# for-the-juan/SpGEMM

Hardware: AMD Instinct MI355X
Metric: SpGEMM GFLOPS (fp64, C=A^2) + achieved HBM GB/s fraction, 1/2/4/8 MI355X (higher is better)
Workload: dtype f64

## Files before the change

### spgemm_amd/csrc/tsg_rows.hip

```cpp
#include "tsg_internal.h"
#include "tsg_dev_common.h"

#include <cstdio>
#include <cstdlib>

namespace tsg {

namespace {

constexpr int S16_MAX = 16;
constexpr int RS_MAX = 64;
constexpr int S16_U = 2, S64_U = 2;
constexpr int M0_CAP = 256, M0_RUNS = 62, M0_NT = 64;
constexpr int M1_CAP = 512, M1_RUNS = 124, M1_NT = 128;
constexpr int M2_CAP = 1024, M2_RUNS = 248, M2_NT = 256;
constexpr int M3_CAP = 2048, M3_RUNS = 504, M3_NT = 512;
constexpr int M4_CAP = 4096, M4_RUNS = 512, M4_NT = 1024;
constexpr int W_CH = 32768;
constexpr int NCLS = 8;
constexpr int DR_SMAX = 4096;
constexpr int DR_CH = 16384;
constexpr int DR_GR = 16;
constexpr int DR_GMAX = 8192;
constexpr int BIN_ROWS = 2048;
constexpr int RH_NT = 1024;
constexpr int RH_WORDS = 16384;
constexpr long long RH_SPAN = (long long)RH_WORDS * 64;
constexpr int RH_BLK = 512;
constexpr int RH_NBLK = RH_WORDS / RH_BLK;
constexpr int RH_NGRP = RH_WORDS / 4;
constexpr int RH_PPT = 16;
constexpr int OW_CH = RH_PPT * RH_NT;
constexpr int OW_CV = 2 * RH_WORDS;
constexpr int OW_RUNS = 2 * RH_NT;
static_assert(OW_CH <= RH_WORDS, "one-walk rows: a pass's values fit the bitmap's LDS");

__device__ __forceinline__ u32 lanes_below(u64 b) {
    return __builtin_amdgcn_mbcnt_hi((u32)(b >> 32), __builtin_amdgcn_mbcnt_lo((u32)b, 0u));
}
__device__ __forceinline__ int key_col(u64 k) { return (int)(k >> 32); }

}

#ifdef TSG_ROWS_PROF
__device__ unsigned long long g_rows_prof[3][256][12];
#define RP_INIT unsigned long long rp_acc[12] = {}, rp_t = wall_clock64();
#define RP(k)                                         \
    do {                                              \
        const unsigned long long _t = wall_clock64(); \
        rp_acc[k] += _t - rp_t;                       \
        rp_t = _t;                                    \
    } while (0)
#define RP_DONE(K)                                                          \
    do {                                                                    \
        if (threadIdx.x == 0)                                               \
            for (int _k = 0; _k < 12; ++_k) atomicAdd(&g_rows_prof[K][blockIdx.x & 255][_k], rp_acc[_k]); \
    } while (0)
#else
#define RP_INIT
#define RP(k) \
    do {      \
    } while (0)
#define RP_DONE(K) \
    do {           \
    } while (0)
#endif

struct RowsArgs {
    const int *rpA;
    const double *vA;
    const int2 *ebnd;
    const long long *E;
    const int *Bcol;
    const double *Bval;
    const int4 *list;
    int nrows;
    int *rnnz;
    int *Scol;
    double *Sval;
};

__device__ __forceinline__ void rows_counters_reset(RowsCounters *cls) {
    constexpr int N = sizeof(RowsCounters) / sizeof(int);
    if (blockIdx.x == 0 && threadIdx.x < N) reinterpret_cast<int *>(cls)[threadIdx.x] = 0;
}

__global__ __launch_bounds__(WG) void k_rows_entries(const int *ciA, long nnzA, const int *rpB, int2 *ebnd,
                                                     long long *E, RowsCounters *cls) {
    rows_counters_reset(cls);
    for (long a = (long)blockIdx.x * WG + threadIdx.x; a <= nnzA; a += (long)gridDim.x * WG) {
        if (a == nnzA) {
            E[a] = 0;
            break;
        }
        const int k = ciA[a], b0 = rpB[k], b1 = rpB[k + 1];
        ebnd[a] = make_int2(b0, b1);
        E[a] = b1 - b0;
    }
}

__global__ __launch_bounds__(WG) void k_rows_entries_sum(const int *ciA, long nnzA, const int *rpB, int2 *ebnd,
                                                         long long *E, RowsCounters *cls, long long *part) {
    __shared__ long long red[WAVES];
    const int tid = threadIdx.x;
    rows_counters_reset(cls);
    const long base = (long)blockIdx.x * SCAN_TILE;
    int kk[SCAN_ITEMS];
#pragma unroll
    for (int u = 0; u < SCAN_ITEMS; ++u) {
        const long a = base + u * WG + tid;
        kk[u] = a < nnzA ? ciA[a] : 0;
    }
    int b0[SCAN_ITEMS], b1[SCAN_ITEMS];
#pragma unroll
    for (int u = 0; u < SCAN_ITEMS; ++u) {
        const long a = base + u * WG + tid;
        b0[u] = a < nnzA ? rpB[kk[u]] : 0;
        b1[u] = a < nnzA ? rpB[kk[u] + 1] : 0;
    }
    long long sum = 0;
#pragma unroll
    for (int u = 0; u < SCAN_ITEMS; ++u) {
        const long a = base + u * WG + tid;
        if (a < nnzA) {
            ebnd[a] = make_int2(b0[u], b1[u]);
            E[a] = b1[u] - b0[u];
            sum += b1[u] - b0[u];
        } else if (a == nnzA) {
            E[a] = 0;
        }
    }
    sum = block_sum(sum, red);
    if (tid == 0) part[blockIdx.x] = sum;
}

__device__ __forceinline__ int row_class(long long P, int k) {
    if (P == 0) return -1;
    if (P <= S16_MAX && k <= S16_MAX) return 0;
    if (P <= RS_MAX && k <= RS_MAX) return 1;
    if (P <= M0_CAP && k <= M0_RUNS) return 2;
    if (P <= M1_CAP && k <= M1_RUNS) return 3;
    if (P <= M2_CAP && k <= M2_RUNS) return 4;
    if (P <= M3_CAP && k <= M3_RUNS) return 5;
    if (P <= M4_CAP && k <= M4_RUNS) return 6;
    return 7;
}

__global__ __launch_bounds__(WG) void k_rows_bin(const int *rpA, int m, const long long *E, const long long *Etot,
                                                 int *rnnz, int4 *lists, RowsCounters *cls, long long *soff,
                                                 const int *spart, int snb, int *sflag) {
    __shared__ int gb[NCLS];
    __shared__ long long red64[WAVES];
    constexpr int RPT = BIN_ROWS / WG;
    __shared__ int wcu[RPT][NCLS][WAVES];
    const int tid = threadIdx.x, lane = lane_id(), wv = wave_id();
    const int r0 = blockIdx.x * BIN_ROWS, r1 = min(m, r0 + BIN_ROWS);
    if (blockIdx.x == 0 && tid == 0) {
        cls->products = (unsigned long long)*Etot;
        rnnz[m] = 0;
    }
    if (blockIdx.x == 0 && spart) {
        long long v = 0;
#pragma unroll 8
        for (int i = tid; i < snb; i += WG) v += spart[i];
        v = block_sum(v, red64);
        if (tid == 0 && v != 0) __hip_atomic_store(sflag, 1, __ATOMIC_RELAXED, __HIP_MEMORY_SCOPE_SYSTEM);
    }
    long long hp = 0, pmax = 0, drp = 0, hubr = 0, hbig = 0;
    int cu[RPT];
    int ra0[RPT], ra1[RPT];
#pragma unroll
    for (int u = 0; u < RPT; ++u) {
        const int r = r0 + u * WG + tid;
        ra0[u] = r < r1 ? rpA[r] : 0;
        ra1[u] = r < r1 ? rpA[r + 1] : 0;
    }
    long long e0[RPT], e1[RPT];
#pragma unroll
    for (int u = 0; u < RPT; ++u) {
        e0[u] = E[ra0[u]];
        e1[u] = E[ra1[u]];
    }
#pragma unroll
    for (int u = 0; u < RPT; ++u) {
        const int r = r0 + u * WG + tid;
        cu[u] = -1;
        if (r >= r1) continue;
        const long long P = e1[u] - e0[u];
        const int c = row_class(P, ra1[u] - ra0[u]);
        soff[r] = e0[u];
        cu[u] = c;
        if (c < 0) rnnz[r] = 0;
        hp += c == NCLS - 1 ? P : 0;
        hbig += c == NCLS - 1 && P <= kRowsHubProducts && P > OW_CH ? P - OW_CH : 0;
        pmax = max(pmax, P);
        if (P > kRowsHubProducts) drp += P;
        if (c == NCLS - 1 && ra1[u] - ra0[u] > OW_RUNS) ++hubr;
    }
    hp = block_sum(hp, red64);
    drp = block_sum(drp, red64);
    hubr = block_sum(hubr, red64);
    hbig = block_sum(hbig, red64);
#pragma unroll
    for (int d = 32; d > 0; d >>= 1) pmax = max(pmax, __shfl_xor(pmax, d, 64));
    if (lane == 0) red64[wv] = pmax;
    __syncthreads();
    if (tid == 0) {
        for (int w = 1; w < WAVES; ++w) pmax = max(pmax, red64[w]);
        if (hp) atomicAdd(&cls->hprod, (unsigned long long)hp);
        if (pmax) atomicMax(&cls->pmax, (unsigned long long)pmax);
        if (drp) atomicAdd(&cls->hubprod, (unsigned long long)drp);
        if (hubr) atomicAdd(&cls->hk, (unsigned long long)hubr);
        if (hbig) atomicAdd(&cls->hbig, (unsigned long long)hbig);
    }
    u64 mine[RPT];
#pragma unroll
    for (int u = 0; u < RPT; ++u) {
        mine[u] = 0;
#pragma unroll
        for (int t = 0; t < NCLS; ++t) {
            const u64 bt = __ballot(cu[u] == t);
            if (cu[u] == t) mine[u] = bt;
            if (lane == 0) wcu[u][t][wv] = __popcll(bt);
        }
    }
    __syncthreads();
    if (tid < NCLS) {
        int run = 0;
        for (int u = 0; u < RPT; ++u)
            for (int w = 0; w < WAVES; ++w) {
                const int v = wcu[u][tid][w];
                wcu[u][tid][w] = run;
                run += v;
            }
        gb[tid] = run ? atomicAdd(&cls->ncls[tid], run) : 0;
    }
    __syncthreads();
#pragma unroll
    for (int u = 0; u < RPT; ++u) {
        const int c = cu[u];
        if (c >= 0) {
            const int r = r0 + u * WG + tid;
            lists[(long)c * m + gb[c] + wcu[u][c][wv] + lanes_below(mine[u])] = make_int4(r, ra0[u], ra1[u] - ra0[u], 0);
        }
    }
}

constexpr int OH_NT = 1024, OH_PER = 8, OH_MAX = OH_NT * OH_PER, OH_NB = 64;
__global__ __launch_bounds__(OH_NT) void k_rows_order_h(const long long *E, const int *nrows, int4 *list) {
    __shared__ int cnt[OH_NB];
    const int tid = threadIdx.x;
    const int n = *nrows;
    if (n < 2 || n > OH_MAX) return;
    if (tid < OH_NB) cnt[tid] = 0;
    __syncthreads();
    int4 r[OH_PER];
    int b[OH_PER];
#pragma unroll
    for (int u = 0; u < OH_PER; ++u) {
        const int i = u * OH_NT + tid;
        r[u] = i < n ? list[i] : make_int4(-1, 0, 0, 0);
    }
#pragma unroll
    for (int u = 0; u < OH_PER; ++u)
        if (r[u].x >= 0) {
            const long long P = E[r[u].y + r[u].z] - E[r[u].y];
            b[u] = OH_NB - 1 - (int)min((long long)OH_NB - 1, P >> 10);
            atomicAdd(&cnt[b[u]], 1);
        }
    __syncthreads();
    if (tid < 64) {
        const int v = cnt[tid];
        const int inc = wave_incl_scan_dpp(v);
        cnt[tid] = inc - v;
    }
    __syncthreads();
#pragma unroll
    for (int u = 0; u < OH_PER; ++u)
        if (r[u].x >= 0) list[atomicAdd(&cnt[b[u]], 1)] = r[u];
}

template <int J> __device__ __forceinline__ int row_bcast16(int v) {
    return __builtin_amdgcn_update_dpp(0, v, 0x150 | J, 0xf, 0xf, false);
}
template <int V> struct IntC { static constexpr int value = V; };
template <int J, int N, class F> __device__ __forceinline__ void static_for(F &&f) {
    if constexpr (J < N) {
        f(IntC<J>{});
        static_for<J + 1, N>(f);
    }
}

template <int G, int U>
__global__ __launch_bounds__(WG) void k_rows_small(RowsArgs g) {
    constexpr int RPW = 64 / G;
    __shared__ u64 sk[WAVES][U][64];
    __shared__ double sv[WAVES][U][64];
    const int lane = lane_id(), wv = wave_id(), sl = lane % G, gb = lane - sl;
    const int w0 = (blockIdx.x * WAVES + wv) * RPW * U;
    if (w0 >= g.nrows) return;
    int r[U], a0[U], k[U];
    bool live[U];
    long long base[U];
#pragma unroll
    for (int u = 0; u < U; ++u) {
        const int i = w0 + u * RPW + lane / G;
        live[u] = i < g.nrows;
        r[u] = 0, a0[u] = 0, k[u] = 0;
        if (live[u]) {
            const int4 e = g.list[i];
            r[u] = e.x;
            a0[u] = e.y;
            k[u] = e.z;
        }
    }
    int2 be[U];
    double av[U];
#pragma unroll
    for (int u = 0; u < U; ++u) {
        be[u] = make_int2(0, 0);
        av[u] = 0.0;
        base[u] = 0;
        if (live[u]) base[u] = g.E[a0[u]];
        if (sl < k[u]) {
            be[u] = g.ebnd[a0[u] + sl];
            av[u] = g.vA[a0[u] + sl];
        }
    }
    int P[U], pp[U];
    double ra[U];
#pragma unroll
    for (int u = 0; u < U; ++u) {
        const int len = be[u].y - be[u].x, bs = be[u].x;
        int inc = len;
        inc += dpp_mov<0x111, 0xf>(0, inc);
        inc += dpp_mov<0x112, 0xf>(0, inc);
        inc += dpp_mov<0x114, 0xf>(0, inc);
        inc += dpp_mov<0x118, 0xf>(0, inc);
        if constexpr (G == 64) {
            inc += dpp_mov<0x142, 0xa>(0, inc);
            inc += dpp_mov<0x143, 0xc>(0, inc);
        }
        const int roff = sl < k[u] ? inc - len : INT_MAX;
        int run = 0;
        if constexpr (G == 64) {
            P[u] = __shfl(inc, G - 1, G);
            for (int j = 1; j < k[u]; ++j) run = (__builtin_amdgcn_readlane(roff, j) <= sl) ? j : run;
        } else {
            static_assert(G == 16, "row broadcasts: 16-lane groups");
            P[u] = row_bcast16<15>(inc);
            static_for<1, 16>([&](auto jc) {
                constexpr int j = decltype(jc)::value;
                run = row_bcast16<j>(roff) <= sl ? j : run;
            });
        }
        const int rs = __shfl(roff, run, G), rb = __shfl(bs, run, G);
        ra[u] = __shfl(av[u], run, G);
        pp[u] = rb + sl - rs;
    }
    u64 key[U];
    double x[U];
#pragma unroll
    for (int u = 0; u < U; ++u) {
        key[u] = ~0ull;
        x[u] = 0.0;
        if (sl < P[u]) {
            key[u] = ((u64)(u32)g.Bcol[pp[u]] << 32) | (u32)sl;
            x[u] = g.Bval[pp[u]];
        }
    }
#pragma unroll
    for (int u = 0; u < U; ++u) {
        const u32 khi = (u32)(key[u] >> 32), klo = (u32)key[u];
        int rank = 0;
        if constexpr (G == 64) {
            for (int f = 0; f < P[u]; ++f) {
                const u64 kf = ((u64)(u32)__builtin_amdgcn_readlane((int)khi, f) << 32) |
                               (u32)__builtin_amdgcn_readlane((int)klo, f);
                rank += kf < key[u];
            }
        } else {
            const u64 ku = key[u];
            static_for<0, 16>([&](auto fc) {
                constexpr int f = decltype(fc)::value;
                const u64 kf = ((u64)(u32)row_bcast16<f>((int)khi) << 32) | (u32)row_bcast16<f>((int)klo);
                rank += kf < ku;
            });
        }
        if (sl < P[u]) {
            sk[wv][u][gb + rank] = key[u];
            sv[wv][u][gb + rank] = ra[u] * x[u];
        }
    }
    wave_lds_sync();
    const u64 gm = (G == 64 ? ~0ull : ((1ull << (G & 63)) - 1ull)) << gb;
#pragma unroll
    for (int u = 0; u < U; ++u) {
        int col = -1;
        bool head = false;
        if (sl < P[u]) {
            col = key_col(sk[wv][u][gb + sl]);
            head = sl == 0 || key_col(sk[wv][u][gb + sl - 1]) != col;
        }
        const u64 hb = __ballot(head) & gm;
        if (head) {
            double sm = sv[wv][u][gb + sl];
            for (int j = sl + 1; j < P[u] && key_col(sk[wv][u][gb + j]) == col; ++j) sm += sv[wv][u][gb + j];
            const long long o = base[u] + (long long)lanes_below(hb);
            g.Scol[o] = col;
            g.Sval[o] = sm;
        }
        if (live[u] && sl == 0) g.rnnz[r[u]] = __popcll(hb);
    }
}

template <int U, class T>
__device__ __forceinline__ void search_ilp(const T *a, int (&b)[U], int (&len)[U], const T (&key)[U],
                                           const bool (&ub)[U]) {
    for (;;) {
        bool more = false;
#pragma unroll
        for (int u = 0; u < U; ++u) more |= len[u] > 0;
        if (!more) break;
#pragma unroll
        for (int u = 0; u < U; ++u) {
            const int half = len[u] >> 1, idx = b[u] + half;
            const T v = a[len[u] > 0 ? idx : 0];
            const bool go = len[u] > 0 && (v < key[u] || (ub[u] && v == key[u]));
            b[u] = go ? idx + 1 : b[u];
            len[u] = go ? len[u] - half - 1 : half;
        }
    }
}

template <int D> __device__ __forceinline__ u32 lane_xor(u32 v) {
    if constexpr (D == 1) return (u32)__builtin_amdgcn_mov_dpp((int)v, 0xB1, 0xf, 0xf, false);
    else if constexpr (D == 2) return (u32)__builtin_amdgcn_mov_dpp((int)v, 0x4E, 0xf, 0xf, false);
    else if constexpr (D < 32) return (u32)__builtin_amdgcn_ds_swizzle((int)v, (D << 10) | 0x1f);
    else return (u32)__shfl_xor((int)v, D, 64);
}

__device__ __forceinline__ u32 minmax_sel(u32 a, u32 b, u32 sel) { return min(max(a, b), max(min(a, b), sel)); }
template <int B> __device__ __forceinline__ u32 bit_fill(u32 v) { return (u32)((int)(v << (31 - B)) >> 31); }
constexpr int ilog2_c(int v) { return v <= 1 ? 0 : 1 + ilog2_c(v >> 1); }

template <int K, int J> __device__ __forceinline__ void bitonic_stage(u32 (&x)[4], int lane) {
    if constexpr (J >= 4) {
        constexpr int D = J / 4;
        u32 w = (u32)lane;
        if constexpr (K < 256) w ^= bit_fill<ilog2_c(K / 4)>((u32)lane);
        const u32 sel = bit_fill<ilog2_c(D)>(w);
#pragma unroll
        for (int u = 0; u < 4; ++u) x[u] = minmax_sel(x[u], lane_xor<D>(x[u]), sel);
    } else {
#pragma unroll
        for (int u = 0; u < 4; ++u)
            if ((u & J) == 0) {
                if constexpr (K < 4 || K >= 256) {
                    const bool asc = K < 4 ? (u & K) == 0 : true;
                    const u32 lo = min(x[u], x[u + J]), hi = max(x[u], x[u + J]);
                    x[u] = asc ? lo : hi;
                    x[u + J] = asc ? hi : lo;
                } else {
                    const u32 desc = bit_fill<ilog2_c(K / 4)>((u32)lane);
                    const u32 a = x[u], b = x[u + J];
                    x[u] = minmax_sel(a, b, desc);
                    x[u + J] = minmax_sel(a, b, ~desc);
                }
            }
    }
}
template <int K, int J> __device__ __forceinline__ void bitonic_merge(u32 (&x)[4], int lane) {
    bitonic_stage<K, J>(x, lane);
    if constexpr (J > 1) bitonic_merge<K, J / 2>(x, lane);
}
template <int K> __device__ __forceinline__ void bitonic_sort(u32 (&x)[4], int lane) {
    if constexpr (K > 2) bitonic_sort<K / 2>(x, lane);
    bitonic_merge<K, K / 2>(x, lane);
}
__device__ __forceinline__ void wave_sort256(u32 (&x)[4], int lane, int live) {
    bitonic_sort<64>(x, lane);
    if (live > 64) bitonic_merge<128, 64>(x, lane);
    if (live > 128) bitonic_merge<256, 128>(x, lane);
}

template <int STRIDE>
__device__ __forceinline__ int xwave_merge(u32 (&x)[4], u32 *kb, int lane, int wv, int P, int npow) {
    constexpr int SEG = 256;
    wv = __builtin_amdgcn_readfirstlane(wv);
    npow = __builtin_amdgcn_readfirstlane(npow);
    const int nlive = (__builtin_amdgcn_readfirstlane(P) + SEG - 1) / SEG;
    const bool live = wv < nlive;
    const int e0 = wv * SEG + 4 * lane;
    int src = 0;
    auto cmpx = [&](int pw, int off, bool rev) {
        if (pw >= nlive) return;
        const uint4 y = *reinterpret_cast<const uint4 *>(kb + src * STRIDE + off);
        const u32 yy[4] = {rev ? y.w : y.x, rev ? y.z : y.y, rev ? y.y : y.z, rev ? y.x : y.w};
        const u32 sel = pw < wv ? ~0u : 0u;
#pragma unroll
        for (int u = 0; u < 4; ++u) x[u] = minmax_sel(x[u], yy[u], sel);
    };
    for (int K = 2 * SEG; K <= npow; K <<= 1) {
        if (live) cmpx(wv ^ (K / SEG - 1), e0 ^ (K - 4), true);
        for (int J = K >> 2; J >= SEG; J >>= 1) {
            src ^= 1;
            if (live) *reinterpret_cast<uint4 *>(kb + src * STRIDE + e0) = make_uint4(x[0], x[1], x[2], x[3]);
            __syncthreads();
            if (live) cmpx(wv ^ (J / SEG), e0 ^ J, false);
        }
        if (live) bitonic_merge<256, 128>(x, lane);
        src ^= 1;
        if (live) *reinterpret_cast<uint4 *>(kb + src * STRIDE + e0) = make_uint4(x[0], x[1], x[2], x[3]);
        __syncthreads();
    }
    return src;
}

template <int NT, int CAP, int RUNS>
__global__ __launch_bounds__(NT, NT == 1024 ? 8 : 1) void k_rows_merge(RowsArgs g) {
    constexpr int NW = NT / 64;
    constexpr int IPM = (CAP + NT - 1) / NT | 1;
    constexpr int IB = CAP == 256 ? 8 : CAP == 512 ? 9 : CAP == 1024 ? 10 : CAP == 2048 ? 11 : 12;
    static_assert((1 << IB) == CAP, "CAP: a power of two in [256, 4096]");
    constexpr int SEG = 256;
    static_assert(CAP == 4 * NT, "four positions per thread");
    static_assert(RUNS <= NT, "a thread per A entry");
    __shared__ __align__(16) u32 kp[2][2][CAP];
    __shared__ int roff[RUNS + 1];
    __shared__ int rbs[RUNS];
    __shared__ double rav[RUNS];
    __shared__ int red[2 * NW];
    RP_INIT
    const int tid = threadIdx.x, lane = lane_id(), wv = wave_id();
    const int4 le = g.list[blockIdx.x];
    int2 be = make_int2(0, 0);
    double av = 0.0;
    if (tid < le.z) {
        be = g.ebnd[le.y + tid];
        av = g.vA[le.y + tid];
    }
    const long long base = g.E[le.y];
    double *const V = reinterpret_cast<double *>(kp[1][0]);
    {
        const int r = le.x;
        int k = 0, P = 0;
        {
            const int len = be.y - be.x;
            const u64 b = __ballot(len > 0);
            const int inc = wave_incl_scan_dpp(len);
            if (lane == 63) {
                red[wv] = __popcll(b);
                red[NW + wv] = inc;
            }
            __syncthreads();
            int off = 0, loff = 0;
#pragma unroll
            for (int w = 0; w < NW; ++w) {
                off += w < wv ? red[w] : 0;
                k += red[w];
                loff += w < wv ? red[NW + w] : 0;
                P += red[NW + w];
            }
            if (len > 0) {
                const int d = off + lanes_below(b);
                roff[d] = loff + inc - len;
                rbs[d] = be.x;
                rav[d] = av;
            }
            if (tid == 0) roff[k] = P;
            __syncthreads();
        }
        RP(0);
        const int e0 = wv * SEG + 4 * lane, ne = max(0, min(4, P - e0));
        int c[4] = {0, 0, 0, 0};
        u32 py[4] = {0, 0, 0, 0};
        double xv[4] = {0.0, 0.0, 0.0, 0.0};
        {
            int j = 0;
            if (ne > 0) j = lower_bound_dev(roff, 0, k + 1, e0 + 1) - 1;
            int pa[4] = {0, 0, 0, 0};
            double ra[4] = {0.0, 0.0, 0.0, 0.0}, bv[4] = {0.0, 0.0, 0.0, 0.0};
#pragma unroll
            for (int u = 0; u < 4; ++u)
                if (u < ne) {
                    const int q = e0 + u;
                    while (roff[j + 1] <= q) ++j;
                    pa[u] = rbs[j] + q - roff[j];
                    py[u] = ((u32)j << 16) | (u32)(q - roff[j]);
                    ra[u] = rav[j];
                }
#pragma unroll
            for (int u = 0; u < 4; ++u)
                if (u < ne) {
                    c[u] = g.Bcol[pa[u]];
                    bv[u] = g.Bval[pa[u]];
                }
#pragma unroll
            for (int u = 0; u < 4; ++u) xv[u] = u < ne ? ra[u] * bv[u] : 0.0;
        }
        int clo = INT_MAX, chi = -1;
#pragma unroll
        for (int u = 0; u < 4; ++u)
            if (u < ne) {
                clo = min(clo, c[u]);
                chi = max(chi, c[u]);
            }
        clo = wave_last(wave_incl_dpp(clo, INT_MAX, OpMin{}));
        chi = wave_last(wave_incl_dpp(chi, INT_MIN, OpMax{}));
        if (lane == 0) {
            red[wv] = clo;
            red[NW + wv] = chi;
        }
        __syncthreads();
        clo = red[0];
        chi = red[NW];
#pragma unroll
        for (int w = 1; w < NW; ++w) {
            clo = min(clo, red[w]);
            chi = max(chi, red[NW + w]);
        }
        const bool packed = (u32)(chi - clo) < (1u << (32 - IB)) - 1u;
        int npow = SEG;
        while (npow < P) npow <<= 1;
        u32 x[4] = {~0u, ~0u, ~0u, ~0u};
        if (packed) {
#pragma unroll
            for (int u = 0; u < 4; ++u) x[u] = u < ne ? ((u32)(c[u] - clo) << IB) | (u32)(e0 + u) : ~0u;
            if (ne > 0) {
                reinterpret_cast<double4 *>(V)[e0 >> 2] = make_double4(xv[0], xv[1], xv[2], xv[3]);
            }
            const int live = __builtin_amdgcn_readfirstlane(P - wv * SEG);
            if (live > 0) {
                wave_sort256(x, lane, live);
                *reinterpret_cast<uint4 *>(kp[0][0] + e0) = make_uint4(x[0], x[1], x[2], x[3]);
            }
        } else {
#pragma unroll
            for (int u = 0; u < 4; ++u)
                if (u < ne) {
                    kp[0][0][e0 + u] = (u32)c[u];
                    kp[0][1][e0 + u] = py[u];
                }
        }
        __syncthreads();
        RP(1);
        int src = 0;
        if (packed) src = xwave_merge<CAP>(x, kp[0][0], lane, wv, P, npow);
        const int ipt = ((P + NT - 1) / NT) | 1;
        const int q0 = min(P, tid * ipt), q1 = min(P, q0 + ipt), nq = q1 - q0;
        if (!packed) {
            const int *const bd = roff;
            const int nb = k;
            int j0 = 0;
            if (nq > 0) j0 = lower_bound_dev(roff, 0, k + 1, q0 + 1) - 1;
            for (int lw = 0; (1 << lw) < nb; ++lw) {
                const u32 *ik = kp[src][0], *ip = kp[src][1];
                u32 *ok = kp[src ^ 1][0], *op = kp[src ^ 1][1];
                int pr = j0 >> (lw + 1);
                for (int q = q0; q < q1;) {
                    while (bd[min((pr + 1) << (lw + 1), nb)] <= q) ++pr;
                    const int ps = bd[pr << (lw + 1)];
                    const int pm = bd[min((2 * pr + 1) << lw, nb)];
                    const int pe = bd[min((pr + 1) << (lw + 1), nb)];
                    const int la = pm - ps, lb = pe - pm, qq = q - ps;
                    int lo = max(0, qq - lb), hi = min(qq, la);
                    while (lo < hi) {
                        const int t = (lo + hi) >> 1;
                        if (ik[ps + t] <= ik[pm + qq - t - 1]) lo = t + 1; else hi = t;
                    }
                    int ia = lo, ib = qq - lo;
                    u32 ka = ia < la ? ik[ps + ia] : ~0u, kbv = ib < lb ? ik[pm + ib] : ~0u;
                    const int qe = min(q1, pe);
                    for (; q < qe; ++q) {
                        const bool ta = ka <= kbv;
                        ok[q] = ta ? ka : kbv;
                        op[q] = ta ? ps + ia : pm + ib;
                        ia += ta;
                        ib += !ta;
                        const u32 kn = ik[ta ? ps + ia : pm + ib];
                        const bool live = ta ? ia < la : ib < lb;
                        ka = ta ? (live ? kn : ~0u) : ka;
                        kbv = ta ? kbv : (live ? kn : ~0u);
                    }
                }
#pragma unroll
                for (int u = 0; u < IPM; ++u)
                    if (u < nq) op[q0 + u] = ip[op[q0 + u]];
                __syncthreads();
                src ^= 1;
            }
        }
        RP(2);
        int nh = 0;
        const int np = packed ? max(0, min(4, P - e0)) : 0;
        double xs[4] = {0.0, 0.0, 0.0, 0.0};
        u32 hd = 0;
        const u32 *const sk = packed ? kp[0][src] : kp[src][0];
        double *const vb = reinterpret_cast<double *>(kp[src ^ 1][0]);
        if (packed) {
            const u32 prev = e0 > 0 && np > 0 ? sk[e0 - 1] : ~0u;
#pragma unroll
            for (int u = 0; u < 4; ++u)
                if (u < np) {
                    xs[u] = V[x[u] & (CAP - 1)];
                    const u32 pk = u ? x[u - 1] : prev;
                    hd |= (e0 + u == 0 || (x[u] >> IB) != (pk >> IB)) ? 1u << u : 0u;
                }
            nh = __popc(hd);
        } else {
            const u32 *sp = kp[src][1];
            int pa[IPM] = {};
            double ra[IPM] = {};
#pragma unroll
            for (int u = 0; u < IPM; ++u)
                if (u < nq) {
                    const u32 key = sk[q0 + u];
                    const u32 pj = sp[q0 + u];
                    const int ru = (int)(pj >> 16);
                    pa[u] = rbs[ru] + (int)(pj & 0xffffu);
                    ra[u] = rav[ru];
                    nh += (q0 + u == 0 || key != sk[q0 + u - 1]);
                }
            double xx[IPM] = {};
#pragma unroll
            for (int u = 0; u < IPM; ++u)
                if (u < nq) xx[u] = ra[u] * g.Bval[pa[u]];
#pragma unroll
            for (int u = 0; u < IPM; ++u)
                if (u < nq) vb[q0 + u] = xx[u];
        }
        const int inc = wave_incl_scan_dpp(nh);
        if (lane == 63) red[wv] = inc;
        __syncthreads();
        RP(3);
        int o = inc - nh, tot = 0;
#pragma unroll
        for (int w = 0; w < NW; ++w) {
            o += w < wv ? red[w] : 0;
            tot += red[w];
        }
        if (tid == 0) g.rnnz[r] = tot;
        if (packed) {
#pragma unroll
            for (int u = 0; u < 4; ++u)
                if (hd >> u & 1u) {
                    const u32 col = x[u] >> IB;
// ... 1730 lines not shown
```

Baseline: 120.0.

## Use in-register bitonic sort on packed 32-bit keys for small-row SpGEMM

In the small-row kernel, products are now sorted by column with a register bitonic network over 32-bit keys. Each key packs the column offset from the group minimum with the lane index, and the network replaces the O(P) rank-counting loop over 64-bit keys. If the group's column span does not fit the packed width, it falls back to the old rank sort. The multiply by the A value moves before the sort, and for 16-lane groups the output-offset load is deferred until after the sort so its latency overlaps. The cost is extra min/max reductions and a shuffle to permute values.

```diff
diff --git a/spgemm_amd/csrc/tsg_rows.hip b/spgemm_amd/csrc/tsg_rows.hip
--- a/spgemm_amd/csrc/tsg_rows.hip
+++ b/spgemm_amd/csrc/tsg_rows.hip
@@ -291,6 +291,29 @@
     }
 }
 
+template <int D> __device__ __forceinline__ u32 lane_xor(u32 v) {
+    if constexpr (D == 1) return (u32)__builtin_amdgcn_mov_dpp((int)v, 0xB1, 0xf, 0xf, false);
+    else if constexpr (D == 2) return (u32)__builtin_amdgcn_mov_dpp((int)v, 0x4E, 0xf, 0xf, false);
+    else if constexpr (D < 32) return (u32)__builtin_amdgcn_ds_swizzle((int)v, (D << 10) | 0x1f);
+    else return (u32)__shfl_xor((int)v, D, 64);
+}
+
+__device__ __forceinline__ u32 minmax_sel(u32 a, u32 b, u32 sel) { return min(max(a, b), max(min(a, b), sel)); }
+template <int B> __device__ __forceinline__ u32 bit_fill(u32 v) { return (u32)((int)(v << (31 - B)) >> 31); }
+constexpr int ilog2_c(int v) { return v <= 1 ? 0 : 1 + ilog2_c(v >> 1); }
+
+template <int G, int K, int J> __device__ __forceinline__ void group_sort_merge(u32 &x, int sl) {
+    u32 w = (u32)sl;
+    if constexpr (K < G) w ^= bit_fill<ilog2_c(K)>((u32)sl);
+    x = minmax_sel(x, lane_xor<J>(x), bit_fill<ilog2_c(J)>(w));
+    if constexpr (J > 1) group_sort_merge<G, K, J / 2>(x, sl);
+}
+template <int G, int K = G> __device__ __forceinline__ void group_sort(u32 &x, int sl) {
+    if constexpr (K > 2) group_sort<G, K / 2>(x, sl);
+    group_sort_merge<G, K, K / 2>(x, sl);
+}
+constexpr int SK_LB = 6;
+
 template <int G, int U>
 __global__ __launch_bounds__(WG) void k_rows_small(RowsArgs g) {
     constexpr int RPW = 64 / G;
@@ -321,7 +344,7 @@
         be[u] = make_int2(0, 0);
         av[u] = 0.0;
         base[u] = 0;
-        if (live[u]) base[u] = g.E[a0[u]];
+        if (G == 64 && live[u]) base[u] = g.E[a0[u]];
         if (sl < k[u]) {
             be[u] = g.ebnd[a0[u] + sl];
             av[u] = g.vA[a0[u] + sl];
@@ -358,29 +381,60 @@
         ra[u] = __shfl(av[u], run, G);
         pp[u] = rb + sl - rs;
     }
-    u64 key[U];
+    int kc[U];
     double x[U];
 #pragma unroll
     for (int u = 0; u < U; ++u) {
-        key[u] = ~0ull;
+        kc[u] = -1;
         x[u] = 0.0;
         if (sl < P[u]) {
-            key[u] = ((u64)(u32)g.Bcol[pp[u]] << 32) | (u32)sl;
+            kc[u] = g.Bcol[pp[u]];
             x[u] = g.Bval[pp[u]];
         }
     }
 #pragma unroll
+    for (int u = 0; u < U; ++u) x[u] *= ra[u];
+#pragma unroll
     for (int u = 0; u < U; ++u) {
-        const u32 khi = (u32)(key[u] >> 32), klo = (u32)key[u];
+        const u32 khi = (u32)kc[u], klo = sl < P[u] ? (u32)sl : ~0u;
+        const u64 key = ((u64)khi << 32) | klo;
+        const bool has = sl < P[u];
+        int clo = has ? (int)khi : INT_MAX, chi = has ? (int)khi : 0;
+        if constexpr (G == 64) {
+            clo = wave_last(wave_incl_dpp(clo, INT_MAX, OpMin{}));
+            chi = wave_last(wave_incl_dpp(chi, 0, OpMax{}));
+        } else {
+            clo = min(clo, dpp_mov<0x111, 0xf>(INT_MAX, clo));
+            clo = min(clo, dpp_mov<0x112, 0xf>(INT_MAX, clo));
+            clo = min(clo, dpp_mov<0x114, 0xf>(INT_MAX, clo));
+            clo = row_bcast16<15>(min(clo, dpp_mov<0x118, 0xf>(INT_MAX, clo)));
+            chi = max(chi, dpp_mov<0x111, 0xf>(0, chi));
+            chi = max(chi, dpp_mov<0x112, 0xf>(0, chi));
+            chi = max(chi, dpp_mov<0x114, 0xf>(0, chi));
+            chi = row_bcast16<15>(max(chi, dpp_mov<0x118, 0xf>(0, chi)));
+        }
+        bool packed = chi - clo < (1 << (32 - SK_LB)) - 1;
+        if constexpr (G < 64) packed = __all(packed);
+        if (packed) {
+            u32 kx = has ? ((u32)((int)khi - clo) << SK_LB) | (u32)sl : ~0u;
+            group_sort<G>(kx, sl);
+            const int src = (int)(kx & (u32)(G - 1));
+            const double pv = __shfl(x[u], src, G);
+            if (has) {
+                sk[wv][u][gb + sl] = ((u64)(u32)((int)(kx >> SK_LB) + clo) << 32) | (u32)src;
+                sv[wv][u][gb + sl] = pv;
+            }
+            continue;
+        }
         int rank = 0;
         if constexpr (G == 64) {
             for (int f = 0; f < P[u]; ++f) {
                 const u64 kf = ((u64)(u32)__builtin_amdgcn_readlane((int)khi, f) << 32) |
                                (u32)__builtin_amdgcn_readlane((int)klo, f);
-                rank += kf < key[u];
+                rank += kf < key;
             }
         } else {
-            const u64 ku = key[u];
+            const u64 ku = key;
             static_for<0, 16>([&](auto fc) {
                 constexpr int f = decltype(fc)::value;
                 const u64 kf = ((u64)(u32)row_bcast16<f>((int)khi) << 32) | (u32)row_bcast16<f>((int)klo);
@@ -388,9 +442,14 @@
             });
         }
         if (sl < P[u]) {
-            sk[wv][u][gb + rank] = key[u];
-            sv[wv][u][gb + rank] = ra[u] * x[u];
-        }
+            sk[wv][u][gb + rank] = key;
+            sv[wv][u][gb + rank] = x[u];
+        }
+    }
+    if constexpr (G < 64) {
+#pragma unroll
+        for (int u = 0; u < U; ++u)
+            if (live[u]) base[u] = g.E[a0[u]];
     }
     wave_lds_sync();
     const u64 gm = (G == 64 ? ~0ull : ((1ull << (G & 63)) - 1ull)) << gb;
@@ -432,17 +491,6 @@
         }
     }
 }
-
-template <int D> __device__ __forceinline__ u32 lane_xor(u32 v) {
-    if constexpr (D == 1) return (u32)__builtin_amdgcn_mov_dpp((int)v, 0xB1, 0xf, 0xf, false);
-    else if constexpr (D == 2) return (u32)__builtin_amdgcn_mov_dpp((int)v, 0x4E, 0xf, 0xf, false);
-    else if constexpr (D < 32) return (u32)__builtin_amdgcn_ds_swizzle((int)v, (D << 10) | 0x1f);
-    else return (u32)__shfl_xor((int)v, D, 64);
-}
-
-__device__ __forceinline__ u32 minmax_sel(u32 a, u32 b, u32 sel) { return min(max(a, b), max(min(a, b), sel)); }
-template <int B> __device__ __forceinline__ u32 bit_fill(u32 v) { return (u32)((int)(v << (31 - B)) >> 31); }
-constexpr int ilog2_c(int v) { return v <= 1 ? 0 : 1 + ilog2_c(v >> 1); }
 
 template <int K, int J> __device__ __forceinline__ void bitonic_stage(u32 (&x)[4], int lane) {
     if constexpr (J >= 4) {
```

Measured after the change: 122.3, median of 6. 1.9% higher.
